# minghanz/bts

Measured on AMD Instinct MI355X. Metric: depth frames/sec at B=16, 352x1216 KITTI input, higher is better.
Workload: dtype f32; 1 GPU; BtsModel.forward (encoder+decoder), densenet161_bts, B=16 per GPU, 3x352x1216 fp32 (BASELINE.json configs[1]); batch_per_gpu=16, global_batch=16, image=352x1216, parallelism=dp1 batch-sharded, RCCL weight broadcast once, hipgraph=True, sub_batch_streams=4, fill_frames=16, encoder_backend=hip, weights=random-init encoder + PCG64(0) synthetic decoder

## Files before the change

bts_amd/_lib.py:

```python
from __future__ import annotations

import ctypes as C
import os
import threading
from typing import Any, Dict, NamedTuple, Optional, Tuple

_HERE = os.path.dirname(os.path.abspath(__file__))
LIB_PATH = os.path.join(_HERE, "libbts_hip.so")

ABI_VERSION = 17


class ConvDesc(C.Structure):
    _fields_ = [
        ("x", C.c_void_p), ("x_pix_stride", C.c_long), ("c_in_ld", C.c_int), ("k_pad", C.c_int),
        ("B", C.c_int), ("h_in", C.c_int), ("w_in", C.c_int), ("up", C.c_int),
        ("ksize", C.c_int), ("dil", C.c_int), ("stride", C.c_int), ("pad", C.c_int),
        ("w", C.c_void_p), ("c_out", C.c_int), ("c_out_pad", C.c_int),
        ("pre_scale", C.c_void_p), ("pre_shift", C.c_void_p), ("pre_relu", C.c_int),
        ("e1_scale", C.c_void_p), ("e1_shift", C.c_void_p), ("act", C.c_int),
        ("e2_scale", C.c_void_p), ("e2_shift", C.c_void_p),
        ("y", C.c_void_p), ("y_pix_stride", C.c_long), ("y_nchw", C.c_int),
        ("subpixel", C.c_int), ("y2", C.c_void_p), ("y2_pix_stride", C.c_long),
        ("splitk_ws", C.c_void_p), ("splitk_ws_floats", C.c_long),
# ... 56 lines not shown

_vp, _i, _l64, _f = C.c_void_p, C.c_int, C.c_long, C.c_float
_pi, _pl, _pvp = C.POINTER(C.c_int), C.POINTER(C.c_long), C.POINTER(C.c_void_p)
_conv, _wgrad = C.POINTER(ConvDesc), C.POINTER(ConvWgradDesc)

ABI: Dict[str, Entry] = {
    "bts_hip_abi_version": _query(_i),
    "bts_hip_error_string": _query(C.c_char_p, _i),
    "bts_lpg_fwd_f32": _launch(_vp, _i, _i, _i, _i, _vp, _vp, _vp, plan=(10, "lpg")),
    "bts_lpg_bwd_f32": _launch(_vp, _vp, _i, _i, _i, _i, _vp, _vp),
    "bts_lpg_fused_fwd_f32": _launch(_vp, _i, _i, _i, _i, _i, _f, _vp, _vp, _i, _l64, _vp, _vp, plan=(4, "lpg_fused")),
    "bts_reduc_fwd_f32": _launch(_vp, _l64, _l64, _i, _i, _vp, _l64, _f, _i, _i, _vp, _vp, plan=(2, "reduc")),
    "bts_reduc_lpg_fwd_f32": _launch(_vp, _l64, _i, _i, _i, _i, _i, _vp, _l64, _f, _i, _vp, _vp, _vp, _vp, _vp, plan=(3, "reduc_lpg")),
    "bts_reduc_bwd_f32": _launch(_vp, _l64, _i, _i, _i, _i, _i, _vp, _l64, _vp, _l64, _f, _i, _vp, _vp, _l64, _vp, _vp, _vp),
    "bts_reduc_bwd_max_waves": _query(_l64, _i, _i, _i),
    "bts_conv_fwd_f32": _launch(_conv, _vp, plan=(1, "conv")),
    "bts_upconv_combine_f32": _launch(_vp, _l64, _i, _i, _i, _i, _vp, _vp, _i, _vp, _l64, _vp, plan=(11, "upconv_combine")),
    "bts_upconv_up9_fwd_f32": _launch(_vp, _l64, _i, _i, _i, _i, _vp, _i, _vp, _vp, _i, _vp, _l64, _vp, plan=(12, "upconv_up9")),
    "bts_upconv_up9_plan": _query(_i, _i, _i, _i, _i, _i, _i, _pi, _pi, _pl),
    "bts_conv_tail_bf16_fwd_f32": _launch(_vp, _l64, _i, _i, _i, _i, _vp, _vp, _vp, _i, _i, _i, _vp, _vp, _i, _vp, _l64, _vp,
                                          plan=(13, "conv_tail_bf16")),
    "bts_conv_tail_bf16_plan": _query(_i, _i, _i, _i, _i, _i, _i, _pi, _pl),
    "bts_conv_tail_wino_fwd_f32": _launch(_vp, _l64, _i, _i, _i, _i, _vp, _vp, _vp, _vp, _vp, _vp, _i, _i, _i, _vp, _vp,
                                          plan=(14, "conv_tail_wino")),
    "bts_conv_tail_wino_plan": _query(_i, _i, _i, _i, _i, _i, _i, _i, _pi, _pi, _pl),
    "bts_conv_grouped_fwd_f32": _launch(_vp, _l64, _i, _i, _i, _i, _i, _vp, _vp, _vp, _i, _vp, _l64, _vp),
    "bts_conv_grouped_plan": _query(_i, _i, _i, _i, _i, _i, _i, _pi, _pi, _pl),
    "bts_conv_grouped_wgrad_f32": _launch(_vp, _l64, _vp, _l64, _i, _i, _i, _i, _i, _vp, _vp, _l64, _vp),
    "bts_conv_grouped_wgrad_plan": _query(_i, _i, _i, _i, _i, _i, _l64, _pi, _pl),
    "bts_conv1x1_bf16_fwd_f32": _launch(_vp, _l64, _l64, _i, _vp, _i, _i, _i, _vp, _vp, _i, _vp, _vp, _i, _vp, _l64, _vp),
    "bts_conv1x1_bf16_plan": _query(_i, _i, _i, _i, _i, _i, _pi, _pi, _pl),
    "bts_conv_plan_f32": _query(_i, _conv, _pi, _pi, _pi),
    "bts_conv_plan_ksteps_f32": _query(_i, _conv, _pl, _pl),
    "bts_conv_wgrad_f32": _launch(_wgrad, _vp),
    "bts_conv_wgrad_plan_f32": _query(_i, _wgrad, _pi, _pi, _pl, _pl),
    "bts_conv_wgrad_batch_table_bytes": _query(_l64, _i),
    "bts_conv_wgrad_batch_plan_f32": _query(_i, _wgrad, _i, _pvp, _pl, _i, _l64, _vp, C.POINTER(ConvWgradBatchItem)),
    "bts_conv_wgrad_batch_f32": _launch(_vp, _vp, _i, _pvp, _i, _vp, _vp),
    "bts_upconv_dgrad_f32": _launch(_vp, _l64, _i, _i, _i, _i, _vp, _i, _vp, _l64, _i, _i, _vp, _l64, _vp),
    "bts_upconv_dgrad_plan": _query(_i, _i, _i, _i, _i, _i, _i, _i, _l64, _pi, _pi, _pi),
    "bts_upconv_wgrad_f32": _launch(_vp, _l64, _i, _i, _i, _i, _vp, _l64, _i, _vp, _vp, _l64, _vp),
    "bts_upconv_wgrad_plan_f32": _query(_i, _i, _i, _i, _i, _i, _l64, _pi, _pi, _pl, _pl),
    "bts_upconv_train_pack_blocks": _query(_l64, _l64, _l64, _l64, _l64),
    "bts_upconv_train_pack_f32": _launch(_vp, _i, _l64, _vp),
    "bts_pack_weights_blocks": _query(_l64, _l64, _l64),
    "bts_pack_weights_f32": _launch(_vp, _i, _l64, _vp),
    "bts_pack_wino_floats": _query(_l64, _i, _i, _i, _i),
    "bts_pack_wino_f32": _launch(_vp, _i, _l64, _i, _i, _i, _vp, _vp),
    "bts_bn_train_ws_floats": _query(_l64, _l64, _i),
    "bts_bn_train_stats_f32": _launch(_vp, _l64, _l64, _i, _vp, _vp, _f, _f, _vp, _vp, _vp, _l64, _vp, _vp, _vp, _vp, _vp),
    "bts_bn_apply_nhwc_f32": _launch(_vp, _l64, _l64, _i, _vp, _vp, _i, _vp, _l64, _vp),
    "bts_bn_train_bwd_f32": _launch(_vp, _l64, _vp, _l64, _l64, _i, _vp, _vp, _vp, _vp, _i, _vp, _l64, _vp, _vp, _vp, _l64, _vp),
    "bts_nchw_to_nhwc_f32": _launch(_vp, _i, _i, _l64, _vp, _l64, _i, _vp, plan=(5, "nchw_to_nhwc")),
    "bts_nhwc_to_nchw_f32": _launch(_vp, _l64, _i, _i, _l64, _vp, _vp, plan=(6, "nhwc_to_nchw")),
    "bts_pack_planes_f32": _launch(_vp, _vp, _vp, _vp, _i, _l64, _vp, _l64, _vp),
    "bts_maxpool3x3s2_nhwc_f32": _launch(_vp, _l64, _i, _i, _i, _i, _vp, _l64, _vp, _l64, _vp, plan=(7, "maxpool")),
    "bts_bn_relu_avgpool2_nhwc_f32": _launch(_vp, _l64, _i, _i, _i, _i, _vp, _vp, _vp, _l64, _vp, plan=(8, "avgpool")),
    "bts_get_depth_f32": _launch(_vp, _vp, _i, _i, _i, _i, _f, _vp, _vp, _vp, plan=(9, "get_depth")),
    "bts_eval_ws_doubles": _query(_l64, _i, _i, _i),
    "bts_eval_depth_metrics_f32": _launch(_vp, _i, _i, _i, _vp, _i, _i, _i, _i, _f, _f, _i, _i, _i, _i, _vp, _l64, _vp, _vp, _vp),
    "bts_depth_loss_ws_doubles": _query(_l64, _l64),
    "bts_depth_loss_fwd_f32": _launch(_vp, _vp, _vp, _f, _l64, _i, _f, _vp, _l64, _vp, _vp, _vp),
    "bts_depth_loss_bwd_f32": _launch(_vp, _vp, _vp, _f, _l64, _i, _f, _vp, _vp, _vp, _vp),
    "bts_adamw_table_bytes": _query(_l64, _i),
    "bts_adamw_flat_span": _query(_l64),
    "bts_adamw_plan_f32": _query(_i, _vp, _i, _vp, _pl, _vp),
# ... 95 lines not shown
```

bts_amd/conv_plan.py:

```python
from __future__ import annotations

import ctypes as C
from collections import namedtuple
from enum import IntEnum, IntFlag

from . import _lib
from ._lib import ConvDesc

class Family(IntEnum):
    ROW, HALO, HALO_TAIL, WIDE_1X1, STEM, HALO_EMU, WINO, ROW_BF16, HALO_BF16 = range(9)


FAMILY_MASK = 15


class Flag(IntFlag):
    SPLITK, W8, DIL = 16, 32, 64


Plan = namedtuple("Plan", "rc family bm bn splitk w8 dil kind issued dense")


def query(desc: ConvDesc, ksteps: bool = False) -> Plan:
    lib = _lib.load_real()
    bm, bn, kind = C.c_int(0), C.c_int(0), C.c_int(0)
    rc = lib.bts_conv_plan_f32(C.byref(desc), C.byref(bm), C.byref(bn), C.byref(kind))
    issued = dense = None
    if ksteps:
        i, d = C.c_long(0), C.c_long(0)
        rc2 = lib.bts_conv_plan_ksteps_f32(C.byref(desc), C.byref(i), C.byref(d))
        assert rc2 == rc, (rc, rc2)
        issued, dense = i.value, d.value
    k = kind.value
    return Plan(rc, Family(k & FAMILY_MASK), bm.value, bn.value, bool(k & Flag.SPLITK), bool(k & Flag.W8),
                bool(k & Flag.DIL), k, issued, dense)


def kernel_name(plan: Plan, nchw: bool, subpixel: bool) -> str:
    f, lay, k = plan.family, "nchw" if nchw else "nhwc", 2 if subpixel else 3
    if f in (Family.ROW, Family.ROW_BF16):
        return "conv_fwd_kernel<%d,%d,%s%s%s>" % (plan.bm, plan.bn, lay, ",splitk" if plan.splitk else "",
                                                 ",bf16" if f == Family.ROW_BF16 else "")
    if f in (Family.HALO, Family.HALO_TAIL):
        return "conv_halo_kernel<%d,k%d,%s%s%s%s>" % (plan.bn, k, lay, ",tail" if f == Family.HALO_TAIL else "",
                                                     ",w8" if plan.w8 else "", ",dil" if plan.dil else "")
    if f in (Family.HALO_EMU, Family.HALO_BF16):
        return "conv_halo_emu_kernel<%d,k%d%s>" % (plan.bn, k, ",bf16" if f == Family.HALO_BF16 else "")
    if f == Family.WIDE_1X1:
        return "conv1x1_kernel<%d,%d>" % (plan.bn, plan.bm // 32)
    return {Family.STEM: "conv_stem_kernel<%d>", Family.WINO: "conv_wino_kernel<%d>"}[f] % plan.bn


def tail_wino_kernel_name() -> str:
    return "conv_wino_tail_kernel<32>"


def tail_bf16_kernel_name(bn: int) -> str:
    return "conv_tail_bf16_kernel<%d>" % bn


def wide_1x1_bf16_kernel_name(bn: int = 192) -> str:
    return "conv1x1_bf16_kernel<%d>" % bn


def grouped_kernel_name(cg: int) -> str:
    return "conv_grouped_kernel<%d>" % cg


def grouped_wgrad_kernel_name(cg: int) -> str:
    return "conv_grouped_wgrad_kernel<%d>" % cg


def round_up(v: int, m: int) -> int:
    return (v + m - 1) // m * m


def conv_out_hw(h: int, w: int, ksize: int, dil: int, stride: int, pad: int, up: int):
    return ((h * up + 2 * pad - dil * (ksize - 1) - 1) // stride + 1,
            (w * up + 2 * pad - dil * (ksize - 1) - 1) // stride + 1)


def geometry_desc(B: int, h: int, w: int, c_in_ld: int, c_out: int, ksize: int, dil: int = 1, stride: int = 1,
                  pad=None, up: int = 1, subpixel: bool = False, n_bundles: int = 0, n_tail: int = 0, nchw: bool = False,
                  fill_frames: int = 0, precision: int = 0, x_pix_stride=None, y_pix_stride=None, c_out_pad=None,
                  fake_pointers: bool = False) -> ConvDesc:
# ... 19 lines not shown
```

bts_amd/csrc/conv_mfma.hip:

```cpp
#include <hip/hip_runtime.h>
#include <stdint.h>
#include <stdlib.h>
#include <type_traits>
#include <algorithm>
#include "common.h"

namespace {

constexpr int BK = 32;

struct ConvKnobs {
    int precision;
    int fill_frames;
    int wino;
    int tapskip;
    int k1x1;
    int halo_dil;
};
inline long env_long(const char* name, long dflt) { const char* v = getenv(name); return v ? atol(v) : dflt; }
const ConvKnobs& knobs() {
    static const ConvKnobs k = {(int)env_long("BTS_CONV_PRECISION", -1),
                                (int)(env_long("BTS_CONV_FILL_FRAMES", 8) > 0 ? env_long("BTS_CONV_FILL_FRAMES", 8) : 8),
                                (int)env_long("BTS_CONV_WINO", 1), (int)env_long("BTS_CONV_TAPSKIP", 1),
                                (int)env_long("BTS_CONV_1X1", 1), (int)env_long("BTS_CONV_HALO_DIL", 1)};
    return k;
}

inline bool nhwc_view_ok(const void* p, long pix_stride, int channels) {
    return p != nullptr && !((uintptr_t)p & 15) && !(pix_stride & 3) && pix_stride >= channels;
}
inline bool act_e2_ok(int act, const float* e2_scale, const float* e2_shift) {
    return (e2_scale == nullptr) == (e2_shift == nullptr) && act >= 0 && act <= 2;
}
inline bool fits_u32(double elements) { return elements < 4294967296.0; }
inline bool resolve_declaration(int fill_frames, int precision, int* ff, int* prec) {
    if (fill_frames < 0 || fill_frames > 4096) return false;
    *ff = fill_frames > 0 ? fill_frames : knobs().fill_frames;
    *prec = knobs().precision >= 0 ? knobs().precision : precision;
    return true;
}
template <int MF> struct LdsLd { static constexpr int value = MF == 32 ? 36 : 40; };

struct ConvArgs {
    const float* x; long x_pix_stride; int c_in_ld; int k_pad;
    int B, h_in, w_in, ups;
    int ksize, dil, stride, pad;
    int subpix;
    int k_flat;
    unsigned magic_c, magic_ks;
    const float* w; int c_out, c_out_pad;
    const float* pre_scale; const float* pre_shift; int pre_relu;
    const float* e1_scale; const float* e1_shift; int act;
    const float* e2_scale; const float* e2_shift;
    float* y; long y_pix_stride;
    float* y2; long y2_pix_stride;
    int H, W;
    int Hs, Ws;
    long M;
    int n_ntiles;
    int tiles_per_class;
    int ksplit, its_per_split, ws_ld;
    float* ws;
    int n_classes, bundled;
    const float* res; long res_pix_stride;
    const float* tail[4];
    int n_tail;
    int fill_frames;
    int halo_single_a;
    int tapskip;
    const float* w_wino;
    const void* w_split;
    int stagger;
};

__host__ __device__ inline unsigned long long tile_tapmask(int H, int W, int Hs, int Ws, int ksize, int dil, int pad_y, int pad_x,
                                                           long M, long m0, int bm) {
    const unsigned HW = (unsigned)(H * W);
    const long mend = m0 + bm < M ? m0 + bm : M;
    const unsigned mf = (unsigned)m0, ml = (unsigned)(mend - 1);
    const unsigned b0 = mf / HW, b1 = ml / HW;
    const unsigned yx0 = mf - b0 * HW, yx1 = ml - b1 * HW;
    const int y0 = (int)(yx0 / (unsigned)W), y1 = (int)(yx1 / (unsigned)W);
    const int x0 = (int)yx0 - y0 * W, x1 = (int)yx1 - y1 * W;
    const bool one_frame = b0 == b1, one_row = one_frame && y0 == y1;
    const int ylo = one_frame ? y0 : 0, yhi = one_frame ? y1 : H - 1;
    const int xlo = one_row ? x0 : 0, xhi = one_row ? x1 : W - 1;
    unsigned long long mask = 0;
    for (int t = 0; t < ksize * ksize; ++t) {
        const int ky = t / ksize, kx = t - ky * ksize;
        const int dy = ky * dil - pad_y, dx = kx * dil - pad_x;
        const int ya = ylo > -dy ? ylo : -dy, yb = yhi < Hs - 1 - dy ? yhi : Hs - 1 - dy;
        const int xa = xlo > -dx ? xlo : -dx, xb = xhi < Ws - 1 - dx ? xhi : Ws - 1 - dx;
        if (ya <= yb && xa <= xb) mask |= 1ull << t;
    }
    return mask ? mask : 1ull;
}

__device__ __forceinline__ float apply_act(float v, int act) {
    if (act == 1) return fmaxf(v, 0.f);
    if (act == 2) return elu1(v);
    if (act == 3) return sigmoid1(v);
    return v;
}


// ... 866 lines not shown
    ConvArgs a{};
    ConvRun r{(hipStream_t)stream, plan, false, 0, 0};
    if (const int rc = conv_args(d, even_ok, a, r); rc != 0) return rc;
    return conv_choose(a, r);
}

int conv_plan(const bts_conv_desc* d, bool even_ok, ConvChoice& c) {
    c = ConvChoice{BTS_CONV_KIND_ROW, 0, 0, 1};
    const int rc = conv_dispatch(d, nullptr, even_ok, &c);
    if (c.ksplit > 1) c.kind |= BTS_CONV_FLAG_SPLITK;
    return rc;
}

}

extern "C" int bts_conv_fwd_f32(const bts_conv_desc* d, bts_stream_t stream) { return conv_dispatch(d, stream); }

extern "C" int bts_conv_plan_f32(const bts_conv_desc* d, int* bm, int* bn, int* kind) {
    if (!d || !bm || !bn || !kind) return BTS_ERR_INVALID;
    ConvChoice c;
    const int rc = conv_plan(d, false, c);
    *bm = c.bm; *bn = c.bn; *kind = c.kind;
    return rc;
}

extern "C" int bts_conv_plan_ksteps_f32(const bts_conv_desc* d, long* issued, long* dense) {
    if (!d || !issued || !dense) return BTS_ERR_INVALID;
    ConvChoice c;
    const int rc = conv_plan(d, false, c);
    *issued = c.ksteps_issued; *dense = c.ksteps_dense;
    return rc;
}

extern "C" int bts_upconv_up9_plan(int h, int w, int c_in, int c_out, int precision, int fill_frames, int* bm, int* bn,
                                   long* workgroups) {
    int ff, prec;
    if (!bm || !bn || !workgroups || !resolve_declaration(fill_frames, precision, &ff, &prec)) return BTS_ERR_INVALID;
    long wgs = 0;
    const bool ok = up9_eligible(h, w, c_in, c_out, prec, ff, &wgs);
    *bm = ok ? UP9_WY * UP9_WX : 0; *bn = ok ? 32 : 0; *workgroups = ok ? wgs : 0;
    return 0;
}

extern "C" int bts_upconv_up9_fwd_f32(const float* x, long x_pix_stride, int B, int h, int w, int c_in, const float* u, int c_out,
                                      const float* e2_scale, const float* e2_shift, int act, float* y, long y_pix_stride,
                                      bts_stream_t stream) {
    if (!x || !u || !y || B <= 0 || h <= 0 || w <= 0 || c_in <= 0 || c_out <= 0) return BTS_ERR_INVALID;
    if ((c_in % BK) || (c_out % 32)) return BTS_ERR_UNSUPPORTED;
    if (!nhwc_view_ok(x, x_pix_stride, c_in) || y_pix_stride < c_out || ((uintptr_t)u & 15) || ((uintptr_t)y & 3)) return BTS_ERR_INVALID;
    if (!act_e2_ok(act, e2_scale, e2_shift)) return BTS_ERR_INVALID;
    if (!fits_u32((double)B * h * w * (double)x_pix_stride) || (double)h * w >= 2147483648.0 ||
        !fits_u32((double)(2 * w + 64) * (double)y_pix_stride)) return BTS_ERR_UNSUPPORTED;
    Up9Args a;
    a.x = x; a.x_pix_stride = x_pix_stride; a.B = B; a.H = h; a.W = w; a.c_in = c_in;
    a.u = u; a.c_out = c_out; a.e2_scale = e2_scale; a.e2_shift = e2_shift; a.act = act;
    a.y = y; a.y_pix_stride = y_pix_stride;
    double fill;
    up9_grid(h, w, &a.n_ty, &a.n_tx, &fill);
    a.n_ntiles = c_out / 32;
    const long nwg = (long)B * a.n_ty * a.n_tx * a.n_ntiles;
    a.ntiles = (int)nwg;
    return conv_launch<conv_up9_kernel<32>>(launch_on(stream), ConvChoice{}, BTS_ERR_UNSUPPORTED, nwg, nwg, 256, 0, a);
}

extern "C" int bts_conv_tail_bf16_plan(int h, int w, int c_main, int c_out, int n_tail, int fill_frames, int* bn, long* workgroups) {
    int ff, prec;
// ... 221 lines not shown
```

bts_amd/csrc/conv_wino.inc:

```
constexpr int WINO_PLD = 36;
constexpr int WINO_PPIX = 10 * 18;

__device__ __forceinline__ int wino_v_off(int row, int chunk16) { return row * 128 + (((chunk16 ^ (row >> 1)) & 7) << 4); }

template <int BN, bool TAIL = false>
constexpr int wino_lds_bytes() {
    constexpr int v = 2 * 16 * 32 * 128 + WINO_PPIX * WINO_PLD * 4;
    constexpr int m = 16 * 32 * 68 * 4 + (TAIL ? WINO_PPIX * 16 + 9 * BN * 16 : 0);
    return v > m ? v : m;
}

template <int BN, bool TAIL = false>
__global__ __launch_bounds__(512, 2) void conv_wino_kernel(const ConvArgs a) {
    constexpr bool MF16 = BN == 48;
    constexpr int NTL = MF16 ? 3 : BN / 32;
    constexpr int NGRP = MF16 ? 4 : 8;
    constexpr int TY = 4, TX = 8;
    constexpr int V_BUF = 16 * 32 * 128;
    constexpr int PW = 18;
    constexpr int RPP = 64, PA = (WINO_PPIX + RPP - 1) / RPP;
    typedef float acc_t __attribute__((ext_vector_type(16)));
    typedef float f32x2 __attribute__((ext_vector_type(2)));
    extern __shared__ __attribute__((aligned(16))) char smem_raw[];
    char* const Vs = smem_raw;
    float* const Ps = reinterpret_cast<float*>(smem_raw + 2 * V_BUF);

    const int tid = threadIdx.x;
    const int wv = __builtin_amdgcn_readfirstlane(tid >> 6), lane = tid & 63;
    const int li = lane & 31, lh = lane >> 5;
    const int c_main = TAIL ? a.c_in_ld - 4 : a.c_in_ld;
    const int nchunks = c_main / BK;
    const int n_tx = (a.W + 2 * TX - 1) / (2 * TX), n_ty = (a.H + 2 * TY - 1) / (2 * TY);
    const int ntiles = a.tiles_per_class;

    const int lrow = tid >> 3, lk = (tid & 7) * 4;
    unsigned abase[PA];
    [[maybe_unused]] unsigned pbase[TAIL ? PA : 1];
    unsigned inimg = 0, inpatch = 0;
    int n0 = 0, bfr = 0, y0 = 0, x0 = 0;
    auto decode = [&](int bid) {
        const int swz = xcd_swizzle(bid, ntiles);
        const int mt_idx = swz / a.n_ntiles, nt_idx = swz - mt_idx * a.n_ntiles;
        n0 = nt_idx * BN;
        bfr = mt_idx / (n_tx * n_ty);
        const int trem = mt_idx - bfr * (n_tx * n_ty);
        const int tyi = trem / n_tx;
        y0 = tyi * 2 * TY; x0 = (trem - tyi * n_tx) * 2 * TX;
        inimg = 0; inpatch = 0;
#pragma unroll
        for (int p = 0; p < PA; ++p) {
            const int pix = p * RPP + lrow;
            const int pyy = pix / PW, pxx = pix - pyy * PW;
            const int gy = y0 - 1 + pyy, gx = x0 - 1 + pxx;
            const bool inp = pix < WINO_PPIX;
            const bool ok = inp && (unsigned)gy < (unsigned)a.H && (unsigned)gx < (unsigned)a.W;
            const int yc = min(max(gy, 0), a.H - 1), xc = min(max(gx, 0), a.W - 1);
            if constexpr (TAIL) pbase[p] = (unsigned)bfr * (unsigned)(a.H * a.W) + (unsigned)(yc * a.W + xc);
            abase[p] = ((unsigned)bfr * (unsigned)(a.H * a.W) + (unsigned)(yc * a.W + xc)) * (unsigned)a.x_pix_stride + (unsigned)lk;
            inimg |= (ok ? 1u : 0u) << p;
            inpatch |= (inp ? 1u : 0u) << p;
        }
    };
    int bid = blockIdx.x;
    decode(bid);
    const bool has_pre = a.pre_scale != nullptr;
    const float* const psrc = has_pre ? a.pre_scale : a.w;
    const float* const bsrc = has_pre ? a.pre_shift : a.w;
    f32x4 pin[PA], ps4 = {1.f, 1.f, 1.f, 1.f}, pb4 = {0.f, 0.f, 0.f, 0.f};
    auto load_patch = [&](int chunk) {
        const unsigned cs = (unsigned)(chunk * BK);
#pragma unroll
        for (int p = 0; p < PA; ++p) pin[p] = *reinterpret_cast<const f32x4*>(a.x + (abase[p] + cs));
        ps4 = *reinterpret_cast<const f32x4*>(psrc + (cs + lk));
        pb4 = *reinterpret_cast<const f32x4*>(bsrc + (cs + lk));
    };
    auto store_patch = [&](int chunk) {
        f32x4 s4 = ps4, b4 = pb4;
        asm volatile("" : "+v"(s4), "+v"(b4));
#pragma unroll
        for (int p = 0; p < PA; ++p) {
            f32x4 v = pin[p];
            asm volatile("" : "+v"(v));
            if (has_pre) v = v * s4 + b4;
            if (a.pre_relu) { v.x = fmaxf(v.x, 0.f); v.y = fmaxf(v.y, 0.f); v.z = fmaxf(v.z, 0.f); v.w = fmaxf(v.w, 0.f); }
            const bool ok = (inimg >> p) & 1u;
            v.x = ok ? v.x : 0.f; v.y = ok ? v.y : 0.f; v.z = ok ? v.z : 0.f; v.w = ok ? v.w : 0.f;
            if ((inpatch >> p) & 1u) *reinterpret_cast<f32x4*>(Ps + (p * RPP + lrow) * WINO_PLD + lk) = v;
        }
    };
    const int tau = tid >> 4, cp = tid & 15;
    const int ty = tau >> 3, tx = tau & 7;
    const float* const pwin = Ps + ((2 * ty) * PW + 2 * tx) * WINO_PLD + 2 * cp;
    const int v_wr = wino_v_off(tau, cp >> 1) + (cp & 1) * 8;
    auto transform_store = [&](char* vbuf) {
        f32x2 d[16];
#pragma unroll
        for (int r = 0; r < 4; ++r)
#pragma unroll
            for (int c = 0; c < 4; ++c) d[4 * r + c] = *reinterpret_cast<const f32x2*>(pwin + (r * PW + c) * WINO_PLD);
        f32x2 t[16];
#pragma unroll
        for (int c = 0; c < 4; ++c) {
            t[0 * 4 + c] = d[0 * 4 + c] - d[2 * 4 + c];
            t[1 * 4 + c] = d[1 * 4 + c] + d[2 * 4 + c];
            t[2 * 4 + c] = d[2 * 4 + c] - d[1 * 4 + c];
            t[3 * 4 + c] = d[1 * 4 + c] - d[3 * 4 + c];
        }
#pragma unroll
        for (int r = 0; r < 4; ++r) {
            const f32x2 v0 = t[r * 4 + 0] - t[r * 4 + 2];
            const f32x2 v1 = t[r * 4 + 1] + t[r * 4 + 2];
            const f32x2 v2 = t[r * 4 + 2] - t[r * 4 + 1];
            const f32x2 v3 = t[r * 4 + 1] - t[r * 4 + 3];
            *reinterpret_cast<f32x2*>(vbuf + (4 * r + 0) * 4096 + v_wr) = v0;
            *reinterpret_cast<f32x2*>(vbuf + (4 * r + 1) * 4096 + v_wr) = v1;
            *reinterpret_cast<f32x2*>(vbuf + (4 * r + 2) * 4096 + v_wr) = v2;
            *reinterpret_cast<f32x2*>(vbuf + (4 * r + 3) * 4096 + v_wr) = v3;
        }
    };

    constexpr int GPC = MF16 ? 2 : 4;
    const int n_ct = MF16 ? a.c_out / 16 : a.c_out_pad / 32;
    const f32x4* ubase = nullptr;
    const size_t xi_stride = (size_t)nchunks * n_ct * (GPC * 64), chunk_stride = (size_t)n_ct * (GPC * 64);
    auto ufrag = [&](int e, int chunk, int j, int g) -> f32x4 { return ubase[e * xi_stride + chunk * chunk_stride + j * (GPC * 64) + g * 64]; };

    acc_t acc[2][MF16 ? 1 : NTL];
    f32x4 acc16[2][2][MF16 ? NTL : 1];
    int a_off[4];
#pragma unroll
    for (int g = 0; g < 4; ++g) a_off[g] = MF16 ? wino_v_off(16 * (g >> 1) + (lane & 15), 4 * (g & 1) + (lane >> 4)) : wino_v_off(li, 2 * g + lh);
    const bool late = wv >= 4;
// ... 38 lines not shown
            }
            if constexpr (MF16) {
                f32x4 fa[2];
#pragma unroll
                for (int i = 0; i < 2; ++i) fa[i] = *reinterpret_cast<const f32x4*>(cur + (2 * wv + e) * 4096 + a_off[2 * i + g]);
#pragma unroll
                for (int q = 0; q < 4; ++q)
#pragma unroll
                    for (int i = 0; i < 2; ++i)
#pragma unroll
                        for (int j = 0; j < NTL; ++j)
                            acc16[e][i][j] = __builtin_amdgcn_mfma_f32_16x16x4f32(fa[i][q], ub[grp & 1][j][q], acc16[e][i][j], 0, 0, 0);
            } else {
                const f32x4 fa = *reinterpret_cast<const f32x4*>(cur + (2 * wv + e) * 4096 + a_off[g]);
#pragma unroll
                for (int q = 0; q < 4; ++q)
#pragma unroll
                    for (int j = 0; j < NTL; ++j)
                        acc[e][j] = __builtin_amdgcn_mfma_f32_32x32x2f32(fa[q], ub[grp & 1][j][q], acc[e][j], 0, 0, 0);
            }
            if (grp == 0) __syncthreads();
            if (grp == (late ? NGRP / 2 : 1) && more) transform_store(nxt);
        }
        __syncthreads();
    }
    float* const Ms = reinterpret_cast<float*>(smem_raw);
    constexpr int M_LD = 68;
    const int cq = tid & 15;
    const bool has_e1 = a.e1_scale != nullptr, has_e2 = a.e2_scale != nullptr;
    constexpr int NPASS = MF16 ? 1 : (NTL + 1) / 2;
    [[maybe_unused]] float* const Ts = reinterpret_cast<float*>(smem_raw + 16 * 32 * M_LD * 4);
    [[maybe_unused]] f32x4* const Wt = reinterpret_cast<f32x4*>(smem_raw + 16 * 32 * M_LD * 4 + WINO_PPIX * 16);
    if constexpr (TAIL) {
        static_assert(wino_lds_bytes<BN, true>() <= 160 * 1024, "tail patch and weights fit behind the exchange buffer");
        for (int i = tid; i < 9 * BN; i += 512) {
            const int tap = i / BN, ch = i - tap * BN;
            Wt[i] = *reinterpret_cast<const f32x4*>(a.w + ((size_t)(n0 + ch) * a.k_pad + tap * a.c_in_ld + c_main));
        }
        if (lk == 0) {
#pragma unroll
            for (int p = 0; p < PA; ++p) {
                f32x4 v = f32x4{a.tail[0][pbase[p]], a.tail[1][pbase[p]], a.tail[2][pbase[p]], a.tail[3][pbase[p]]};
                const bool ok = (inimg >> p) & 1u;
                v.x = ok ? v.x : 0.f; v.y = ok && a.n_tail > 1 ? v.y : 0.f; v.z = ok && a.n_tail > 2 ? v.z : 0.f; v.w = ok && a.n_tail > 3 ? v.w : 0.f;
                if ((inpatch >> p) & 1u) *reinterpret_cast<f32x4*>(Ts + (p * RPP + lrow) * 4) = v;
            }
        }
    }
    const int cy0 = y0, cx0 = x0, cbfr = bfr, cn0 = n0;
    const int nbid = bid + (int)gridDim.x;
    const bool have_next = nbid < ntiles;
    constexpr bool EARLY = BN <= 64;
    if (EARLY && have_next) { decode(nbid); load_patch(0); }
#pragma unroll
    for (int p = 0; p < NPASS; ++p) {
        if (p > 0) __syncthreads();
        if constexpr (MF16) {
#pragma unroll
            for (int e = 0; e < 2; ++e)
#pragma unroll
                for (int i = 0; i < 2; ++i)
#pragma unroll
                    for (int j = 0; j < NTL; ++j)
#pragma unroll
                        for (int r = 0; r < 4; ++r)
                            Ms[((2 * wv + e) * 32 + 16 * i + 4 * (lane >> 4) + r) * M_LD + j * 16 + (lane & 15)] = acc16[e][i][j][r];
        } else {
#pragma unroll
            for (int e = 0; e < 2; ++e)
#pragma unroll
                for (int jj = 0; jj < 2; ++jj) {
                    const int j = 2 * p + jj;
                    if (j < NTL) {
#pragma unroll
                        for (int r = 0; r < 16; ++r) {
                            const int trow = (r & 3) + 8 * (r >> 2) + 4 * lh;
                            Ms[((2 * wv + e) * 32 + trow) * M_LD + jj * 32 + li] = acc[e][j][r];
                        }
                    }
                }
        }
        __syncthreads();
        const int nch = cn0 + p * 64 + 4 * cq;
        if (4 * cq < (MF16 ? 48 : (NTL - 2 * p >= 2 ? 64 : 32))) {
            f32x4 m[16];
#pragma unroll
            for (int xi = 0; xi < 16; ++xi) m[xi] = *reinterpret_cast<const f32x4*>(Ms + (xi * 32 + tau) * M_LD + 4 * cq);
            f32x4 s[8];
#pragma unroll
            for (int c = 0; c < 4; ++c) {
                s[0 * 4 + c] = m[0 * 4 + c] + m[1 * 4 + c] + m[2 * 4 + c];
                s[1 * 4 + c] = m[1 * 4 + c] - m[2 * 4 + c] - m[3 * 4 + c];
            }
            [[maybe_unused]] f32x4 tacc[4];
            if constexpr (TAIL) {
#pragma unroll
                for (int o = 0; o < 4; ++o) tacc[o] = f32x4{0.f, 0.f, 0.f, 0.f};
                const f32x4* const wt = Wt + (p * 64 + 4 * cq);
                if (a.n_tail == 1) {
                    float tvx[16];
#pragma unroll
                    for (int r = 0; r < 4; ++r)
#pragma unroll
                        for (int c = 0; c < 4; ++c) tvx[4 * r + c] = Ts[((2 * ty + r) * PW + 2 * tx + c) * 4];
#pragma unroll
                    for (int tap = 0; tap < 9; ++tap) {
                        float wk[4];
#pragma unroll
                        for (int k = 0; k < 4; ++k) wk[k] = wt[tap * BN + k].x;
#pragma unroll
                        for (int o = 0; o < 4; ++o)
#pragma unroll
                            for (int k = 0; k < 4; ++k)
                                tacc[o][k] = fmaf(wk[k], tvx[4 * ((o >> 1) + tap / 3) + (o & 1) + tap % 3], tacc[o][k]);
                    }
                } else {
#pragma unroll 3
                    for (int tap = 0; tap < 9; ++tap) {
                        f32x4 wk[4];
#pragma unroll
                        for (int k = 0; k < 4; ++k) wk[k] = wt[tap * BN + k];
#pragma unroll
                        for (int o = 0; o < 4; ++o) {
                            const f32x4 tv = *reinterpret_cast<const f32x4*>(Ts + ((2 * ty + (o >> 1) + tap / 3) * PW + 2 * tx + (o & 1) + tap % 3) * 4);
#pragma unroll
                            for (int k = 0; k < 4; ++k) {
                                float sacc = tacc[o][k];
                                sacc = fmaf(wk[k].x, tv.x, sacc);
                                sacc = fmaf(wk[k].y, tv.y, sacc);
                                if (a.n_tail > 2) sacc = fmaf(wk[k].z, tv.z, sacc);
                                if (a.n_tail > 3) sacc = fmaf(wk[k].w, tv.w, sacc);
                                tacc[o][k] = sacc;
                            }
                        }
                    }
                }
            }
            if (EARLY && p == 0 && have_next) {
#pragma unroll
                for (int q = 0; q < PA; ++q) asm volatile("" : "+v"(pin[q]));
                asm volatile("" : "+v"(ps4), "+v"(pb4));
            }
            f32x4 e1s = {1.f, 1.f, 1.f, 1.f}, e1b = {0.f, 0.f, 0.f, 0.f}, e2s = e1s, e2b = e1b;
            const bool cin_range = nch + 3 < a.c_out_pad;
            if (has_e1 && cin_range) { e1s = *reinterpret_cast<const f32x4*>(a.e1_scale + nch); e1b = *reinterpret_cast<const f32x4*>(a.e1_shift + nch); }
            if (has_e2 && cin_range) { e2s = *reinterpret_cast<const f32x4*>(a.e2_scale + nch); e2b = *reinterpret_cast<const f32x4*>(a.e2_shift + nch); }
#pragma unroll
            for (int oy = 0; oy < 2; ++oy)
#pragma unroll
                for (int ox = 0; ox < 2; ++ox) {
                    f32x4 v = ox == 0 ? s[oy * 4 + 0] + s[oy * 4 + 1] + s[oy * 4 + 2] : s[oy * 4 + 1] - s[oy * 4 + 2] - s[oy * 4 + 3];
                    if constexpr (TAIL) v += tacc[2 * oy + ox];
                    const int y = cy0 + 2 * ty + oy, x = cx0 + 2 * tx + ox;
                    if (y < a.H && x < a.W) {
                        const long pix = ((long)cbfr * a.H + y) * a.W + x;
                        float o[4];
#pragma unroll
                        for (int k = 0; k < 4; ++k) {
                            float t = v[k] * e1s[k] + e1b[k];
                            if (a.res != nullptr && nch + k < a.c_out) t += a.res[pix * a.res_pix_stride + nch + k];
                            t = apply_act(t, a.act);
                            o[k] = t * e2s[k] + e2b[k];
                        }
                        float* yp = a.y + pix * a.y_pix_stride + nch;
                        if (nch + 3 < a.c_out && ((a.y_pix_stride & 3) == 0) && ((reinterpret_cast<uintptr_t>(yp) & 15) == 0)) {
                            *reinterpret_cast<f32x4*>(yp) = f32x4{o[0], o[1], o[2], o[3]};
                        } else {
#pragma unroll
                            for (int k = 0; k < 4; ++k) if (nch + k < a.c_out) yp[k] = o[k];
                        }
                        if (a.y2) {
                            float* y2p = a.y2 + pix * a.y2_pix_stride + nch;
#pragma unroll
                            for (int k = 0; k < 4; ++k) if (nch + k < a.c_out) y2p[k] = o[k];
                        }
                    }
                }
        }
    }
    if (!have_next) break;
    if (!EARLY) { decode(nbid); load_patch(0); }
    __syncthreads();
    bid = nbid;
  }
}

inline bool wino_eligible(const ConvArgs& a, bool nchw) {
    if (a.w_wino == nullptr || nchw || a.subpix || a.bundled || a.ups != 0) return false;
    const int c_main = a.n_tail > 0 ? a.c_in_ld - 4 : a.c_in_ld;
    if (a.ksize != 3 || a.stride != 1 || a.dil != 1 || a.pad != 1 || c_main <= 0 || (c_main % BK) != 0) return false;
    if (((uintptr_t)a.w_wino & 15)) return false;
    const long ntx = (a.W + 15) / 16, nty = (a.H + 7) / 8;
    constexpr double min_fill = 0.70;
    return (double)a.H * a.W / (double)(ntx * 16 * nty * 8) >= min_fill;
}

template <int BN, bool TAIL = false>
int launch_wino(const ConvArgs& a0, const ConvRun& r) {
    ConvArgs a = a0;
    const long n_mtiles = (long)a.B * ((a.H + 7) / 8) * ((a.W + 15) / 16);
    a.n_ntiles = (a.c_out + BN - 1) / BN;
    a.tiles_per_class = (int)(n_mtiles * a.n_ntiles);
    a.ksplit = 1;
    const long nwg = n_mtiles * a.n_ntiles;
    constexpr size_t lds = (size_t)wino_lds_bytes<BN, TAIL>();
    static_assert(lds <= 160 * 1024, "LDS");
    const long R = (nwg + 255) / 256;
    long G = ((nwg + R - 1) / R + 7) & ~7L;
    if (G > nwg) G = nwg;
    return conv_launch<conv_wino_kernel<BN, TAIL>>(r, ConvChoice{BTS_CONV_KIND_WINO, 128, BN, 1}, BTS_ERR_INVALID, nwg, G, 512, lds, a);
}
```

bts_amd/ops.py:

```python
from __future__ import annotations

import ctypes as C
import os
import threading
from typing import List, Optional, Sequence, Tuple

import torch
import torch.nn.functional as F

from . import _lib, conv_plan
from ._lib import BtsHipError, ConvDesc, ConvWgradBatchItem, ConvWgradDesc
from .conv_plan import conv_out_hw, round_up

ACT_NONE, ACT_RELU, ACT_ELU, ACT_SIGMOID = 0, 1, 2, 3


class KernelTrace:

    def __init__(self):
        self.records = []

    def summary(self):
        torch.cuda.synchronize()
        out = {}
# ... 1528 lines not shown
        wsplit_t = (_derived_weight(w_packed, "_bts_split3", split_bf16x3) if d.precision == 1 else
                    _derived_weight(w_packed, "_bts_round1", round_bf16))
        keep.append(wsplit_t)
        d.w_split = wsplit_t.data_ptr()
    if (_WINO and d.precision == 0 and d.ksize == 3 and d.stride == 1 and d.dil == 1 and d.pad == 1 and d.up == 1
            and not d.n_bundles and c_main % 32 == 0 and d.c_in_ld > 4 and not d.y_nchw):
        def make(w):
            d.w_wino = w.data_ptr()
            w._bts_wino_c16 = d.c_out if conv_plan.query(d).bn == 48 else 0
            return pack_wino_weight(w, d.c_in_ld, d.n_tail, c_out16=w._bts_wino_c16)

        uw = _derived_weight(w_packed, "_bts_wino", make, refill=lambda w, out: pack_wino_weight(
            w, d.c_in_ld, d.n_tail, c_out16=getattr(w, "_bts_wino_c16", 0), out=out))
        keep.append(uw)
        d.w_wino = uw.data_ptr()
    return wsplit_t, uw


def _conv_trace_accounting(d: ConvDesc, c_in_real: Optional[int], algo_flops: Optional[float]):
    B, c_in_ld = d.B, d.c_in_ld
    H, W = (2 * d.h_in, 2 * d.w_in) if d.subpixel else conv_out_hw(d.h_in, d.w_in, d.ksize, d.dil, d.stride, d.pad, d.up)
    flops_taps, taps = (9, 4) if d.subpixel else (d.ksize * d.ksize,) * 2
    cin = c_in_real if c_in_real is not None else c_in_ld
    npix_out = B * H * W
    c_out = d.c_out * max(d.n_bundles, 1)
    flops = 2.0 * npix_out * c_out * cin * flops_taps
    if algo_flops is not None:
        flops = float(algo_flops)
    nbytes = 4.0 * (B * d.h_in * d.w_in * cin + npix_out * c_out + flops_taps * c_out * cin)
    plan = conv_plan.query(d, ksteps=True)
    variant = conv_plan.kernel_name(plan, bool(d.y_nchw), bool(d.subpixel))
    xflops = 2.0 * npix_out * c_out * (c_in_ld if d.n_bundles > 1 else cin) * taps
    if plan.family == conv_plan.Family.WINO:
        nwg = B * ((H + 7) // 8) * ((W + 15) // 16) * ((c_out + plan.bn - 1) // plan.bn)
        xflops = 2.0 * nwg * 16 * 32 * plan.bn * c_in_ld
    if plan.dense > 0:
        xflops *= plan.issued / plan.dense
    return variant, flops, nbytes, xflops


_GEOM_FIELDS = ("x_pix_stride", "c_in_ld", "k_pad", "B", "h_in", "w_in", "up", "ksize", "dil", "stride", "pad", "c_out", "c_out_pad",
                "pre_relu", "act", "y_pix_stride", "y_nchw", "subpixel", "y2_pix_stride", "res_pix_stride", "n_bundles", "precision",
                "fill_frames")


def conv_forward(x2d: torch.Tensor, B: int, h_in: int, w_in: int, w_packed: torch.Tensor, c_out: int,
                 ksize: int, dil: int = 1, up: int = 1, c_in_ld: Optional[int] = None,
                 pre: Optional[Tuple[torch.Tensor, torch.Tensor]] = None, pre_relu: bool = False,
                 e1: Optional[Tuple[torch.Tensor, torch.Tensor]] = None, act: int = ACT_NONE,
                 e2: Optional[Tuple[torch.Tensor, torch.Tensor]] = None,
                 y2d: Optional[torch.Tensor] = None, y_nchw: Optional[torch.Tensor] = None,
                 tag: str = "conv", c_in_real: Optional[int] = None, stride: int = 1, pad: Optional[int] = None,
                 y2_2d: Optional[torch.Tensor] = None, subpixel: bool = False,
                 splitk_ws: Optional[torch.Tensor] = None, res2d: Optional[torch.Tensor] = None, n_bundles: int = 1,
                 tail_planes: Optional[Sequence[torch.Tensor]] = None, algo_flops: Optional[float] = None):
    d, out, keep = _conv_describe(x2d, B, h_in, w_in, w_packed, c_out, ksize, dil, up, c_in_ld, pre, pre_relu, e1, act, e2,
                                  y2d, y_nchw, stride, pad, y2_2d, subpixel, splitk_ws, res2d, n_bundles, tail_planes)
    wsplit_t, uw_t = _conv_derived_weights(d, w_packed, keep)
    trace = None
    if _trace is not None:
        kern, flops, nbytes, xflops = _conv_trace_accounting(d, c_in_real, algo_flops)
        trace = (kern, tag, flops, nbytes, xflops)
    tops = torch_ops()
    run = None
    if tops is not None:
        geom = [getattr(d, f) for f in _GEOM_FIELDS]
        (pre_s, pre_b), (e1_s, e1_b), (e2_s, e2_b) = (p if p is not None else (None, None) for p in (pre, e1, e2))
# ... 438 lines not shown
```

include/bts_hip.h:

```cpp
#ifndef BTS_HIP_H_
#define BTS_HIP_H_

#ifdef __cplusplus
extern "C" {
#endif

#define BTS_HIP_ABI_VERSION 17

#define BTS_ERR_INVALID      (-1)
#define BTS_ERR_UNSUPPORTED  (-2)

typedef void* bts_stream_t;

int         bts_hip_abi_version(void);
const char* bts_hip_error_string(int code);

int bts_lpg_fwd_f32(const float* plane_eq, int B, int h, int w, int upratio,
                    float* depth, float* abs_min, bts_stream_t stream);

int bts_lpg_bwd_f32(const float* plane_eq, const float* grad_depth, int B, int h, int w, int upratio,
                    float* grad_plane_eq, bts_stream_t stream);

int bts_lpg_fused_fwd_f32(const float* plane4, int B, int h, int w, int upratio, int normalize,
                          float max_depth, float* depth_scaled,
// ... 89 lines not shown
int bts_conv_tail_wino_plan(int h, int w, int c_main, int c_out, int n_tail, int precision, int fill_frames, int* bm, int* bn,
                            long* workgroups);

int bts_conv_grouped_fwd_f32(const float* x, long x_pix_stride, int B, int h, int w, int c, int groups, const float* w_packed,
                             const float* e1_scale, const float* e1_shift, int act, float* y, long y_pix_stride,
                             bts_stream_t stream);

int bts_conv_grouped_plan(int h, int w, int c, int groups, int precision, int fill_frames, int* bm, int* bn, long* workgroups);

int bts_conv_grouped_wgrad_f32(const float* x, long x_pix_stride, const float* dy, long dy_pix_stride, int B, int h, int w, int c,
                               int groups, float* dw, float* ws, long ws_floats, bts_stream_t stream);

int bts_conv_grouped_wgrad_plan(int B, int h, int w, int c, int groups, long ws_floats, int* splits, long* ws_floats_used);

enum {
    BTS_CONV_KIND_ROW       = 0,
    BTS_CONV_KIND_HALO      = 1,
    BTS_CONV_KIND_HALO_TAIL = 2,
    BTS_CONV_KIND_WIDE_1X1  = 3,
    BTS_CONV_KIND_STEM      = 4,
    BTS_CONV_KIND_HALO_EMU  = 5,
    BTS_CONV_KIND_WINO      = 6,
    BTS_CONV_KIND_ROW_BF16  = 7,
    BTS_CONV_KIND_HALO_BF16 = 8,
    BTS_CONV_KIND_MASK      = 15,
    BTS_CONV_FLAG_SPLITK    = 16,
    BTS_CONV_FLAG_W8        = 32,
    BTS_CONV_FLAG_DIL       = 64
};
int bts_conv_plan_f32(const bts_conv_desc* desc, int* bm, int* bn, int* kind);

int bts_conv_plan_ksteps_f32(const bts_conv_desc* desc, long* issued, long* dense);

typedef struct bts_conv_wgrad_desc {
    const float* x;
    long  x_pix_stride;
    int   c_in;
    const float* dy;
    long  dy_pix_stride;
    int   c_out;
    int   B, h_in, w_in;
    int   up, ksize, dil, stride, pad;
    float* dw;
    float* ws;
    long  ws_floats;
    int   n_bundles;
    const float* pre_scale;
    const float* pre_shift;
    int   pre_relu;
} bts_conv_wgrad_desc;

int bts_conv_wgrad_f32(const bts_conv_wgrad_desc* desc, bts_stream_t stream);

int bts_conv_wgrad_plan_f32(const bts_conv_wgrad_desc* desc, int* bm, int* bn, long* split, long* pix_per_split);

typedef struct bts_conv_wgrad_batch_item {
    int  bm, bn;
    long split;
    long pix_per_split;
    long ws_offset;
} bts_conv_wgrad_batch_item;

long bts_conv_wgrad_batch_table_bytes(int n);
int  bts_conv_wgrad_batch_plan_f32(const bts_conv_wgrad_desc* descs, int n, const void* const* bases, const long* base_bytes,
                                   int n_bases, long ws_floats, void* table_host, bts_conv_wgrad_batch_item* plan );
int  bts_conv_wgrad_batch_f32(const void* table_host, const void* table_dev, int n, const void* const* bases, int n_bases,
// ... 141 lines not shown
```

Before: 492.3 frames/s.

## Use mixed-shape Winograd tiling to cut padded edge tiles

Replaces the uniform 8x16-pixel Winograd tiling with a mixed plan. Full 4x8 tiles cover the interior, and narrower 8x4 or 2x16 tile shapes cover ragged right and bottom edges. The aim is fewer wasted tile computations when H or W is not a multiple of the tile size. A BIG kernel variant with a larger patch buffer handles the 2x16 shape. Tile decode now runs a per-tile plan function, which adds index arithmetic to the kernel prologue.

```diff
diff --git a/bts_amd/_lib.py b/bts_amd/_lib.py
--- a/bts_amd/_lib.py
+++ b/bts_amd/_lib.py
@@ -112,6 +112,7 @@
     "bts_conv1x1_bf16_plan": _query(_i, _i, _i, _i, _i, _i, _pi, _pi, _pl),
     "bts_conv_plan_f32": _query(_i, _conv, _pi, _pi, _pi),
     "bts_conv_plan_ksteps_f32": _query(_i, _conv, _pl, _pl),
+    "bts_conv_wino_tiles": _query(_i, _i, _i, _i, _pi, _i),
     "bts_conv_wgrad_f32": _launch(_wgrad, _vp),
     "bts_conv_wgrad_plan_f32": _query(_i, _wgrad, _pi, _pi, _pl, _pl),
     "bts_conv_wgrad_batch_table_bytes": _query(_l64, _i),
diff --git a/bts_amd/conv_plan.py b/bts_amd/conv_plan.py
--- a/bts_amd/conv_plan.py
+++ b/bts_amd/conv_plan.py
@@ -51,6 +51,17 @@
     return {Family.STEM: "conv_stem_kernel<%d>", Family.WINO: "conv_wino_kernel<%d>"}[f] % plan.bn
 
 
+def wino_tiles(h: int, w: int, tiling: int = -1, want_tiles: bool = False):
+    lib = _lib.load_real()
+    n = lib.bts_conv_wino_tiles(int(h), int(w), int(tiling), None, 0)
+    _lib.check(min(n, 0), "bts_conv_wino_tiles")
+    if not want_tiles:
+        return n
+    buf = (C.c_int * (5 * n))()
+    assert lib.bts_conv_wino_tiles(int(h), int(w), int(tiling), buf, n) == n
+    return n, [tuple(buf[5 * i:5 * i + 5]) for i in range(n)]
+
+
 def tail_wino_kernel_name() -> str:
     return "conv_wino_tail_kernel<32>"
 
diff --git a/bts_amd/csrc/conv_mfma.hip b/bts_amd/csrc/conv_mfma.hip
--- a/bts_amd/csrc/conv_mfma.hip
+++ b/bts_amd/csrc/conv_mfma.hip
@@ -16,13 +16,15 @@
     int tapskip;
     int k1x1;
     int halo_dil;
+    int wino_mixed;
 };
 inline long env_long(const char* name, long dflt) { const char* v = getenv(name); return v ? atol(v) : dflt; }
 const ConvKnobs& knobs() {
     static const ConvKnobs k = {(int)env_long("BTS_CONV_PRECISION", -1),
                                 (int)(env_long("BTS_CONV_FILL_FRAMES", 8) > 0 ? env_long("BTS_CONV_FILL_FRAMES", 8) : 8),
                                 (int)env_long("BTS_CONV_WINO", 1), (int)env_long("BTS_CONV_TAPSKIP", 1),
-                                (int)env_long("BTS_CONV_1X1", 1), (int)env_long("BTS_CONV_HALO_DIL", 1)};
+                                (int)env_long("BTS_CONV_1X1", 1), (int)env_long("BTS_CONV_HALO_DIL", 1),
+                                (int)env_long("BTS_CONV_WINO_MIXED", 1)};
     return k;
 }
 
@@ -71,6 +73,7 @@
     const float* w_wino;
     const void* w_split;
     int stagger;
+    int wino_mixed;
 };
 
 __host__ __device__ inline unsigned long long tile_tapmask(int H, int W, int Hs, int Ws, int ksize, int dil, int pad_y, int pad_x,
@@ -1003,6 +1006,19 @@
     return rc;
 }
 
+extern "C" int bts_conv_wino_tiles(int h, int w, int tiling, int* tiles, int cap) {
+    if (h <= 0 || w <= 0 || tiling < -1 || tiling > 1 || cap < 0 || (tiles == nullptr && cap > 0)) return BTS_ERR_INVALID;
+    if ((long)((h + 7) / 8) * ((w + 15) / 16) > 0x7fffffffL) return BTS_ERR_UNSUPPORTED;
+    const bool mixed = tiling < 0 ? knobs().wino_mixed != 0 : tiling == 1;
+    const int n = wino_plan_tile(h, w, mixed, 0, nullptr);
+    for (int t = 0; t < n && t < cap; ++t) {
+        WinoTile tl;
+        wino_plan_tile(h, w, mixed, t, &tl);
+        tiles[5 * t] = tl.shape; tiles[5 * t + 1] = tl.wy; tiles[5 * t + 2] = tl.wx; tiles[5 * t + 3] = tl.wy_end; tiles[5 * t + 4] = tl.wx_end;
+    }
+    return n;
+}
+
 extern "C" int bts_upconv_up9_plan(int h, int w, int c_in, int c_out, int precision, int fill_frames, int* bm, int* bn,
                                    long* workgroups) {
     int ff, prec;
diff --git a/bts_amd/csrc/conv_wino.inc b/bts_amd/csrc/conv_wino.inc
--- a/bts_amd/csrc/conv_wino.inc
+++ b/bts_amd/csrc/conv_wino.inc
@@ -1,24 +1,54 @@
 constexpr int WINO_PLD = 36;
-constexpr int WINO_PPIX = 10 * 18;
+constexpr int wino_ppix(bool big) { return big ? 6 * 34 : 10 * 18; }
+
+enum { WINO_SHAPE_4x8 = 0, WINO_SHAPE_8x4 = 1, WINO_SHAPE_2x16 = 2 };
+__host__ __device__ __forceinline__ int wino_shape_log2tx(int sh) { return sh == WINO_SHAPE_4x8 ? 3 : (sh == WINO_SHAPE_8x4 ? 2 : 4); }
+__host__ __device__ __forceinline__ int wino_shape_pw(int sh) { return (2 << wino_shape_log2tx(sh)) + 2; }
+
+struct WinoTile { int shape, wy, wx, wy_end, wx_end; };
+__host__ __device__ __forceinline__ int wino_plan_tile(int H, int W, bool mixed, int t, WinoTile* tile) {
+    const int R = (H + 1) / 2, C = (W + 1) / 2;
+    const int u_stride = (C + 7) / 8, u_tiles = ((R + 3) / 4) * u_stride;
+    const int mr = R / 4 * 4, mc = C / 8 * 8, sr = R - mr, sc = C - mc;
+    const int cnt0 = (mr / 4) * (mc / 8);
+    const int cnt1 = sc == 0 ? 0 : (sc <= 4 ? (R + 7) / 8 : (R + 3) / 4);
+    const int cnt2 = sr == 0 ? 0 : (sr <= 2 ? (mc + 15) / 16 : mc / 8);
+    const bool m = mixed && cnt0 + cnt1 + cnt2 < u_tiles;
+    if (tile != nullptr) {
+        if (!m || t < cnt0) {
+            const int st = m ? mc / 8 : u_stride;
+            const int ry = t / st, rx = t - ry * st;
+            *tile = WinoTile{WINO_SHAPE_4x8, 4 * ry, 8 * rx, m ? mr : R, m ? mc : C};
+        } else if (t < cnt0 + cnt1) {
+            const bool narrow = sc <= 4;
+            *tile = WinoTile{narrow ? WINO_SHAPE_8x4 : WINO_SHAPE_4x8, (t - cnt0) * (narrow ? 8 : 4), mc, R, C};
+        } else {
+            const bool low = sr <= 2;
+            *tile = WinoTile{low ? WINO_SHAPE_2x16 : WINO_SHAPE_4x8, mr, (t - cnt0 - cnt1) * (low ? 16 : 8), R, mc};
+        }
+    }
+    return m ? cnt0 + cnt1 + cnt2 : u_tiles;
+}
 
 __device__ __forceinline__ int wino_v_off(int row, int chunk16) { return row * 128 + (((chunk16 ^ (row >> 1)) & 7) << 4); }
 
-template <int BN, bool TAIL = false>
+template <int BN, bool TAIL = false, bool BIG = false>
 constexpr int wino_lds_bytes() {
+    constexpr int WINO_PPIX = wino_ppix(BIG);
     constexpr int v = 2 * 16 * 32 * 128 + WINO_PPIX * WINO_PLD * 4;
     constexpr int m = 16 * 32 * 68 * 4 + (TAIL ? WINO_PPIX * 16 + 9 * BN * 16 : 0);
     return v > m ? v : m;
 }
 
-template <int BN, bool TAIL = false>
+template <int BN, bool TAIL = false, bool BIG = false>
 __global__ __launch_bounds__(512, 2) void conv_wino_kernel(const ConvArgs a) {
+    constexpr int WINO_PPIX = wino_ppix(BIG);
     constexpr bool MF16 = BN == 48;
     constexpr int NTL = MF16 ? 3 : BN / 32;
     constexpr int NGRP = MF16 ? 4 : 8;
-    constexpr int TY = 4, TX = 8;
     constexpr int V_BUF = 16 * 32 * 128;
-    constexpr int PW = 18;
     constexpr int RPP = 64, PA = (WINO_PPIX + RPP - 1) / RPP;
+    constexpr int PA_SMALL = (180 + RPP - 1) / RPP;
     typedef float acc_t __attribute__((ext_vector_type(16)));
     typedef float f32x2 __attribute__((ext_vector_type(2)));
     extern __shared__ __attribute__((aligned(16))) char smem_raw[];
@@ -30,33 +60,45 @@
     const int li = lane & 31, lh = lane >> 5;
     const int c_main = TAIL ? a.c_in_ld - 4 : a.c_in_ld;
     const int nchunks = c_main / BK;
-    const int n_tx = (a.W + 2 * TX - 1) / (2 * TX), n_ty = (a.H + 2 * TY - 1) / (2 * TY);
     const int ntiles = a.tiles_per_class;
+    const int tau = tid >> 4, cp = tid & 15;
 
     const int lrow = tid >> 3, lk = (tid & 7) * 4;
     unsigned abase[PA];
     [[maybe_unused]] unsigned pbase[TAIL ? PA : 1];
     unsigned inimg = 0, inpatch = 0;
-    int n0 = 0, bfr = 0, y0 = 0, x0 = 0;
+    int n0 = 0, bfr = 0, y0 = 0, x0 = 0, sh = 0;
+    int yend = 0, xend = 0;
+    const float* pwin = Ps;
+    int prow = 0;
     auto decode = [&](int bid) {
         const int swz = xcd_swizzle(bid, ntiles);
         const int mt_idx = swz / a.n_ntiles, nt_idx = swz - mt_idx * a.n_ntiles;
         n0 = nt_idx * BN;
-        bfr = mt_idx / (n_tx * n_ty);
-        const int trem = mt_idx - bfr * (n_tx * n_ty);
-        const int tyi = trem / n_tx;
-        y0 = tyi * 2 * TY; x0 = (trem - tyi * n_tx) * 2 * TX;
+        const int ftiles = wino_plan_tile(a.H, a.W, a.wino_mixed != 0, 0, nullptr);
+        bfr = mt_idx / ftiles;
+        WinoTile tl;
+        wino_plan_tile(a.H, a.W, a.wino_mixed != 0, mt_idx - bfr * ftiles, &tl);
+        sh = tl.shape;
+        y0 = 2 * tl.wy; x0 = 2 * tl.wx;
+        yend = min(2 * tl.wy_end, a.H); xend = min(2 * tl.wx_end, a.W);
+        const int l = wino_shape_log2tx(sh), pw = wino_shape_pw(sh);
+        const int npix = BIG && sh == WINO_SHAPE_2x16 ? 6 * 34 : 10 * 18;
+        const int pw_magic = sh == WINO_SHAPE_4x8 ? 3641 : (sh == WINO_SHAPE_8x4 ? 6554 : 1928);
+        pwin = Ps + ((2 * (tau >> l)) * pw + 2 * (tau & ((1 << l) - 1))) * WINO_PLD + 2 * cp;
+        prow = pw * WINO_PLD;
         inimg = 0; inpatch = 0;
 #pragma unroll
         for (int p = 0; p < PA; ++p) {
             const int pix = p * RPP + lrow;
-            const int pyy = pix / PW, pxx = pix - pyy * PW;
+            const int pyy = (pix * pw_magic) >> 16, pxx = pix - pyy * pw;
             const int gy = y0 - 1 + pyy, gx = x0 - 1 + pxx;
-            const bool inp = pix < WINO_PPIX;
+            const bool inp = pix < npix;
             const bool ok = inp && (unsigned)gy < (unsigned)a.H && (unsigned)gx < (unsigned)a.W;
             const int yc = min(max(gy, 0), a.H - 1), xc = min(max(gx, 0), a.W - 1);
             if constexpr (TAIL) pbase[p] = (unsigned)bfr * (unsigned)(a.H * a.W) + (unsigned)(yc * a.W + xc);
             abase[p] = ((unsigned)bfr * (unsigned)(a.H * a.W) + (unsigned)(yc * a.W + xc)) * (unsigned)a.x_pix_stride + (unsigned)lk;
+            if (p >= PA_SMALL && !inp) abase[p] = abase[0];
             inimg |= (ok ? 1u : 0u) << p;
             inpatch |= (inp ? 1u : 0u) << p;
         }
@@ -88,16 +130,13 @@
             if ((inpatch >> p) & 1u) *reinterpret_cast<f32x4*>(Ps + (p * RPP + lrow) * WINO_PLD + lk) = v;
         }
     };
-    const int tau = tid >> 4, cp = tid & 15;
-    const int ty = tau >> 3, tx = tau & 7;
-    const float* const pwin = Ps + ((2 * ty) * PW + 2 * tx) * WINO_PLD + 2 * cp;
     const int v_wr = wino_v_off(tau, cp >> 1) + (cp & 1) * 8;
     auto transform_store = [&](char* vbuf) {
         f32x2 d[16];
 #pragma unroll
         for (int r = 0; r < 4; ++r)
 #pragma unroll
-            for (int c = 0; c < 4; ++c) d[4 * r + c] = *reinterpret_cast<const f32x2*>(pwin + (r * PW + c) * WINO_PLD);
+            for (int c = 0; c < 4; ++c) d[4 * r + c] = *reinterpret_cast<const f32x2*>(pwin + r * prow + c * WINO_PLD);
         f32x2 t[16];
 #pragma unroll
         for (int c = 0; c < 4; ++c) {
@@ -202,7 +241,7 @@
     [[maybe_unused]] float* const Ts = reinterpret_cast<float*>(smem_raw + 16 * 32 * M_LD * 4);
     [[maybe_unused]] f32x4* const Wt = reinterpret_cast<f32x4*>(smem_raw + 16 * 32 * M_LD * 4 + WINO_PPIX * 16);
     if constexpr (TAIL) {
-        static_assert(wino_lds_bytes<BN, true>() <= 160 * 1024, "tail patch and weights fit behind the exchange buffer");
+        static_assert(wino_lds_bytes<BN, true, BIG>() <= 160 * 1024, "tail patch and weights fit behind the exchange buffer");
         for (int i = tid; i < 9 * BN; i += 512) {
             const int tap = i / BN, ch = i - tap * BN;
             Wt[i] = *reinterpret_cast<const f32x4*>(a.w + ((size_t)(n0 + ch) * a.k_pad + tap * a.c_in_ld + c_main));
@@ -217,7 +256,9 @@
             }
         }
     }
-    const int cy0 = y0, cx0 = x0, cbfr = bfr, cn0 = n0;
+    const int cy0 = y0, cx0 = x0, cbfr = bfr, cn0 = n0, cyend = yend, cxend = xend;
+    const int cl = wino_shape_log2tx(sh), cpw = wino_shape_pw(sh);
+    const int ty = tau >> cl, tx = tau & ((1 << cl) - 1);
     const int nbid = bid + (int)gridDim.x;
     const bool have_next = nbid < ntiles;
     constexpr bool EARLY = BN <= 64;
@@ -267,12 +308,13 @@
 #pragma unroll
                 for (int o = 0; o < 4; ++o) tacc[o] = f32x4{0.f, 0.f, 0.f, 0.f};
                 const f32x4* const wt = Wt + (p * 64 + 4 * cq);
+                const float* const tsw = Ts + ((2 * ty) * cpw + 2 * tx) * 4;
                 if (a.n_tail == 1) {
                     float tvx[16];
 #pragma unroll
                     for (int r = 0; r < 4; ++r)
 #pragma unroll
-                        for (int c = 0; c < 4; ++c) tvx[4 * r + c] = Ts[((2 * ty + r) * PW + 2 * tx + c) * 4];
+                        for (int c = 0; c < 4; ++c) tvx[4 * r + c] = tsw[(r * cpw + c) * 4];
 #pragma unroll
                     for (int tap = 0; tap < 9; ++tap) {
                         float wk[4];
@@ -292,7 +334,7 @@
                         for (int k = 0; k < 4; ++k) wk[k] = wt[tap * BN + k];
 #pragma unroll
                         for (int o = 0; o < 4; ++o) {
-                            const f32x4 tv = *reinterpret_cast<const f32x4*>(Ts + ((2 * ty + (o >> 1) + tap / 3) * PW + 2 * tx + (o & 1) + tap % 3) * 4);
+                            const f32x4 tv = *reinterpret_cast<const f32x4*>(tsw + (((o >> 1) + tap / 3) * cpw + (o & 1) + tap % 3) * 4);
 #pragma unroll
                             for (int k = 0; k < 4; ++k) {
                                 float sacc = tacc[o][k];
@@ -322,7 +364,7 @@
                     f32x4 v = ox == 0 ? s[oy * 4 + 0] + s[oy * 4 + 1] + s[oy * 4 + 2] : s[oy * 4 + 1] - s[oy * 4 + 2] - s[oy * 4 + 3];
                     if constexpr (TAIL) v += tacc[2 * oy + ox];
                     const int y = cy0 + 2 * ty + oy, x = cx0 + 2 * tx + ox;
-                    if (y < a.H && x < a.W) {
+                    if (y < cyend && x < cxend) {
                         const long pix = ((long)cbfr * a.H + y) * a.W + x;
                         float o[4];
 #pragma unroll
@@ -365,18 +407,24 @@
     return (double)a.H * a.W / (double)(ntx * 16 * nty * 8) >= min_fill;
 }
 
-template <int BN, bool TAIL = false>
+template <int BN, bool TAIL = false, bool BIG = false>
 int launch_wino(const ConvArgs& a0, const ConvRun& r) {
+    if constexpr (!BIG) {
+        const int R = (a0.H + 1) / 2, C = (a0.W + 1) / 2;
+        const bool mixed = knobs().wino_mixed != 0 && wino_plan_tile(a0.H, a0.W, true, 0, nullptr) < wino_plan_tile(a0.H, a0.W, false, 0, nullptr);
+        if (mixed && (R & 3) >= 1 && (R & 3) <= 2 && C >= 8) return launch_wino<BN, TAIL, true>(a0, r);
+    }
     ConvArgs a = a0;
-    const long n_mtiles = (long)a.B * ((a.H + 7) / 8) * ((a.W + 15) / 16);
+    a.wino_mixed = knobs().wino_mixed != 0;
+    const long n_mtiles = (long)a.B * wino_plan_tile(a.H, a.W, a.wino_mixed != 0, 0, nullptr);
     a.n_ntiles = (a.c_out + BN - 1) / BN;
     a.tiles_per_class = (int)(n_mtiles * a.n_ntiles);
     a.ksplit = 1;
     const long nwg = n_mtiles * a.n_ntiles;
-    constexpr size_t lds = (size_t)wino_lds_bytes<BN, TAIL>();
+    constexpr size_t lds = (size_t)wino_lds_bytes<BN, TAIL, BIG>();
     static_assert(lds <= 160 * 1024, "LDS");
     const long R = (nwg + 255) / 256;
     long G = ((nwg + R - 1) / R + 7) & ~7L;
     if (G > nwg) G = nwg;
-    return conv_launch<conv_wino_kernel<BN, TAIL>>(r, ConvChoice{BTS_CONV_KIND_WINO, 128, BN, 1}, BTS_ERR_INVALID, nwg, G, 512, lds, a);
+    return conv_launch<conv_wino_kernel<BN, TAIL, BIG>>(r, ConvChoice{BTS_CONV_KIND_WINO, 128, BN, 1}, BTS_ERR_INVALID, nwg, G, 512, lds, a);
 }
diff --git a/bts_amd/ops.py b/bts_amd/ops.py
--- a/bts_amd/ops.py
+++ b/bts_amd/ops.py
@@ -1584,7 +1584,7 @@
     variant = conv_plan.kernel_name(plan, bool(d.y_nchw), bool(d.subpixel))
     xflops = 2.0 * npix_out * c_out * (c_in_ld if d.n_bundles > 1 else cin) * taps
     if plan.family == conv_plan.Family.WINO:
-        nwg = B * ((H + 7) // 8) * ((W + 15) // 16) * ((c_out + plan.bn - 1) // plan.bn)
+        nwg = B * conv_plan.wino_tiles(H, W) * ((c_out + plan.bn - 1) // plan.bn)
         xflops = 2.0 * nwg * 16 * 32 * plan.bn * c_in_ld
     if plan.dense > 0:
         xflops *= plan.issued / plan.dense
diff --git a/include/bts_hip.h b/include/bts_hip.h
--- a/include/bts_hip.h
+++ b/include/bts_hip.h
@@ -145,6 +145,8 @@
 
 int bts_conv_plan_ksteps_f32(const bts_conv_desc* desc, long* issued, long* dense);
 
+int bts_conv_wino_tiles(int h, int w, int tiling, int* tiles, int cap);
+
 typedef struct bts_conv_wgrad_desc {
     const float* x;
     long  x_pix_stride;
```

Measured after the change: 495.5 frames/s (median of 6 runs). About the same (+0.6%).
